# Ryan-Yanlong/DREAM-GNN

Measured on AMD Instinct MI355X. Metric: GCMC+FGCN SpMM edges/sec and achieved HBM GB/s at 1/2/4/8 MI355X, higher is better.
Workload: dtype f32

## Files before the change

dream_gnn_amd/csrc/dgmi_owned.hip:

```cpp
#include <hip/hip_runtime.h>
#include <stdint.h>

#include <map>
#include <mutex>
#include <utility>

#include "dgmi_owned_common.h"
#include "dgmi_sliced_common.h"

namespace dgmi {
namespace {

constexpr int kOwnedTouchChunk = 4;
constexpr int kOwnedTouchLead = 8;
constexpr int64_t kOwnedSpinTicks = 3000;
constexpr int64_t kOwnedMinRows = 32768;
constexpr int kOwnedLag = -1;

struct OwnedWork {
  int phase, task, slice, col_round;
  int64_t row0;
  int lds_row, rows;
};

__device__ __forceinline__ OwnedWork owned_decode(const OwnedPlan& pl, int64_t wg, int T, int k, int grp) {
  OwnedWork w;
  w.phase = k / T;
  w.task = k - w.phase * T;
  const OwnedPhase ph = owned_phase(pl, w.phase);
  w.slice = ph.slice;
  w.col_round = ph.col_round;
  const OwnedTask t = owned_task(pl, wg, ph.row_round, w.task, grp);
  w.row0 = t.row0;
  w.lds_row = t.lds_row;
  w.rows = t.rows;
  return w;
}

template <int LPR, int VALS, bool OFF32, int WAVES>
__global__ __launch_bounds__(kWave* WAVES, WAVES == kOwnedWaves ? 4 : 6) void spmm_owned_kernel(
    const int32_t* __restrict__ segptr, const int32_t* __restrict__ indices, const float* __restrict__ X, int64_t ldx,
    const float* __restrict__ dst_scale, float* __restrict__ Y, int64_t ldy, int64_t n_dst, int F, OwnedPlan pl,
    unsigned* __restrict__ arrive, int lag, int64_t spin_ticks, Epilogue ep) {
  constexpr bool MULT = VALS == 2;
  constexpr int kIdMask = MULT ? (int)kMultIdMask : 0x7fffffff;
  extern __shared__ float4 lds_rows[];
  const int lane = threadIdx.x & (kWave - 1);
  const int wave = threadIdx.x >> 6;
  const int grp = lane / LPR, glane = lane % LPR, gbase = grp * LPR;
  const int64_t wg = blockIdx.x;
  const int T = owned_wg_tasks(pl, wg);
  if (T == 0) return;
  int* done = reinterpret_cast<int*>(lds_rows + (size_t)pl.round_rows * LPR);
  int* phase_cnt = done + pl.tasks;
  int* counter = phase_cnt + pl.phases;
  int* open = counter + 1;
  for (int i = threadIdx.x; i < pl.tasks + pl.phases + 2; i += blockDim.x) done[i] = 0;
  __syncthreads();
  const int total = pl.phases * T;
  const int label = (int)(blockIdx.x & 7u);

  if (wave == WAVES - 1) {
    const unsigned n_label = (unsigned)((pl.active - label + 7) >> 3);
    const unsigned* my_arrive = arrive + (size_t)label * pl.phases;
    const int chunks_per_phase = (T + kOwnedTouchChunk - 1) / kOwnedTouchChunk, chunks = pl.phases * chunks_per_phase;
    const int last_gate = lag >= 0 ? pl.phases - 1 : 0;
    int keepalive = 0, touched = 0, opened = 0;
    bool waiting = false;
    uint64_t wait_start = 0;
    while (touched < chunks || opened < last_gate) {
      bool idle = true;
      const int next = __hip_atomic_load(counter, __ATOMIC_RELAXED, __HIP_MEMORY_SCOPE_WORKGROUP);
      if (touched < chunks) {
        const int P = touched / chunks_per_phase, t0 = (touched - P * chunks_per_phase) * kOwnedTouchChunk;
        if (P * T + t0 <= next + kOwnedTouchLead) {
          ++touched;
          idle = false;
          const OwnedPhase ph = owned_phase(pl, P);
          const int64_t in_round = owned_round_rows(pl, wg, ph.row_round);
          const int64_t lds_first = (int64_t)t0 * pl.G * pl.R;
          int64_t lds_last = lds_first + (int64_t)kOwnedTouchChunk * pl.G * pl.R;
          if (lds_last > in_round) lds_last = in_round;
          if (lds_first < lds_last) {
            const int32_t* sp_s = segptr + (int64_t)ph.slice * n_dst;
            const int64_t r_first = owned_task(pl, wg, ph.row_round, t0, 0).row0, r_last = r_first + (lds_last - lds_first);
            const int64_t rp = lane == 0 ? r_first : (lane == 1 ? r_last : r_first + (int64_t)(lane - 1) * 32);
            int v = 0;
            if (rp <= r_last) v = sp_s[rp];
            keepalive ^= v;
            const int e0 = __builtin_amdgcn_readlane(v, 0), e1 = __builtin_amdgcn_readlane(v, 1);
            for (int64_t p = (int64_t)e0 + (int64_t)lane * 32; p < e1; p += (int64_t)kWave * 32) keepalive ^= indices[p];
            asm volatile("" ::"v"(keepalive));
          }
        }
      }
      if (opened < last_gate) {
        const int P = opened + 1, need = P - 1 - lag;
        bool ok = need < 0 || __hip_atomic_load(&my_arrive[need], __ATOMIC_RELAXED, __HIP_MEMORY_SCOPE_AGENT) >= n_label;
        if (!ok && next >= P * T) {
          const uint64_t now = __builtin_amdgcn_s_memrealtime();
          if (!waiting) {
            waiting = true;
            wait_start = now;
          } else if (now - wait_start >= (uint64_t)spin_ticks) {
            ok = true;
          }
        }
        if (ok) {
          opened = P;
          waiting = false;
          idle = false;
          __hip_atomic_store(open, P, __ATOMIC_RELAXED, __HIP_MEMORY_SCOPE_WORKGROUP);
        }
      }
      if (idle) __builtin_amdgcn_s_sleep(2);
    }
    return;
  }

  auto grab = [&]() {
    int k = 0;
    if (lane == 0) k = __hip_atomic_fetch_add(counter, 1, __ATOMIC_RELAXED, __HIP_MEMORY_SCOPE_WORKGROUP);
    return __builtin_amdgcn_readfirstlane(k);
  };
  auto boundaries = [&](int k) {
    if (k >= total) return 0;
    const OwnedWork w = owned_decode(pl, wg, T, k, grp);
    if (w.rows == 0) return 0;
    return segptr[(int64_t)w.slice * n_dst + w.row0 + (glane < w.rows ? glane : w.rows)];
  };
  auto first_ids = [&](int my_b, int rows) {
    const int e_begin = __shfl(my_b, gbase, kWave), e_end = __shfl(my_b, gbase + rows, kWave);
    if (rows == 0 || e_begin >= e_end) return 0;
    return indices[e_begin + glane < e_end ? e_begin + glane : e_begin];
  };

  const uint32_t row_bytes = (uint32_t)ldx * 4u;
  int k = grab();
  int my_b = boundaries(k);
  int nxt_idx = k < total ? first_ids(my_b, owned_decode(pl, wg, T, k, grp).rows) : 0;
  while (k < total) {
    const OwnedWork w = owned_decode(pl, wg, T, k, grp);
    const int k_next = grab();
    const int next_b = boundaries(k_next);
    if (lag >= 0)
      while (__hip_atomic_load(open, __ATOMIC_RELAXED, __HIP_MEMORY_SCOPE_WORKGROUP) < w.phase) __builtin_amdgcn_s_sleep(1);
    while (__hip_atomic_load(&done[w.task], __ATOMIC_ACQUIRE, __HIP_MEMORY_SCOPE_WORKGROUP) < w.phase) __builtin_amdgcn_s_sleep(1);

    const int nr = w.rows;
    int col = (w.col_round * LPR + glane) * 4;
    const bool col_ok = col < F;
    if (!col_ok) col = 0;
    const float* Xc = X + col;
    const uint32_t col_bytes = (uint32_t)col * 4u;
    float4* slot = lds_rows + (size_t)w.lds_row * LPR + glane;
    auto commit = [&](int r, const float4& acc) {
      if (w.slice == 0) {
        slot[r * LPR] = acc;
        return;
      }
      float4 t = slot[r * LPR];
      t.x += acc.x;
      t.y += acc.y;
      t.z += acc.z;
      t.w += acc.w;
      slot[r * LPR] = t;
    };
    auto write_rows = [&]() {
      if (w.slice != kOwnedSlices - 1 || !col_ok) return;
      for (int r = 0; r < nr; ++r) {
        float4 t = slot[r * LPR];
        const int64_t row = w.row0 + r;
        if (dst_scale != nullptr) {
          const float d = dst_scale[row];
          t.x *= d;
          t.y *= d;
          t.z *= d;
          t.w *= d;
        }
        *reinterpret_cast<float4*>(Y + row * ldy + col) = epilogue4(ep, t, row, col);
      }
    };

    if (nr > 0) {
      const int e_begin = __shfl(my_b, gbase, kWave);
      const int e_end = __shfl(my_b, gbase + nr, kWave);
      int r = 0;
      int row_end = __shfl(my_b, gbase + 1, kWave);
      float4 acc = make_float4(0.f, 0.f, 0.f, 0.f);
      for (int base = e_begin; base < e_end; base += LPR) {
        const int n = min(LPR, e_end - base);
        const int my_idx = nxt_idx;
        if (base + LPR < e_end) {
          const int nb = base + LPR;
          nxt_idx = indices[nb + glane < e_end ? nb + glane : nb];
        }
        for (int j = 0; j < n; j += kUnroll) {
          float4 v[kUnroll];
          static_assert(kUnroll == 8 && kMultShift == 28, "eight 4-bit fields, each shifted down from bit 28");
          uint32_t mults = 0;
          auto mult = [&](int u) { return (float)(((mults >> (4 * u)) & (uint32_t)kMultMax) + 1u); };
#pragma unroll
          for (int u = 0; u < kUnroll; ++u) {
            int idx = __shfl(my_idx, gbase + j + u, kWave);
            if (MULT) {
              mults = (mults >> 4) | ((uint32_t)idx & ((uint32_t)kMultMax << kMultShift));
              idx &= kIdMask;
            }
            v[u] = ld_row<OFF32>(X, Xc, idx, ldx, row_bytes, col_bytes);
          }
          if (MULT) asm volatile("" : "+v"(mults));
          if (base + j + kUnroll <= row_end) {
#pragma unroll
            for (int u = 0; u < kUnroll; ++u) {
              if (MULT) {
                const float m = mult(u);
                acc.x = fmaf(m, v[u].x, acc.x);
                acc.y = fmaf(m, v[u].y, acc.y);
                acc.z = fmaf(m, v[u].z, acc.z);
                acc.w = fmaf(m, v[u].w, acc.w);
              } else {
                acc.x += v[u].x;
                acc.y += v[u].y;
                acc.z += v[u].z;
                acc.w += v[u].w;
              }
            }
            continue;
          }
#pragma unroll
          for (int u = 0; u < kUnroll; ++u) {
            const int p = base + j + u;
            if (p < e_end) {
              while (p >= row_end) {
                commit(r, acc);
                acc = make_float4(0.f, 0.f, 0.f, 0.f);
                ++r;
                row_end = __shfl(my_b, gbase + r + 1, kWave);
              }
              if (MULT) {
                const float m = mult(u);
                acc.x = fmaf(m, v[u].x, acc.x);
                acc.y = fmaf(m, v[u].y, acc.y);
                acc.z = fmaf(m, v[u].z, acc.z);
                acc.w = fmaf(m, v[u].w, acc.w);
              } else {
                acc.x += v[u].x;
                acc.y += v[u].y;
                acc.z += v[u].z;
                acc.w += v[u].w;
              }
            }
          }
        }
      }
      for (; r < nr; ++r) {
        commit(r, acc);
        acc = make_float4(0.f, 0.f, 0.f, 0.f);
      }
      write_rows();
    }
    nxt_idx = k_next < total ? first_ids(next_b, owned_decode(pl, wg, T, k_next, grp).rows) : 0;
    __builtin_amdgcn_wave_barrier();
    if (lane == 0) {
      __hip_atomic_store(&done[w.task], w.phase + 1, __ATOMIC_RELEASE, __HIP_MEMORY_SCOPE_WORKGROUP);
      if (lag >= 0) {
        const int finished = __hip_atomic_fetch_add(&phase_cnt[w.phase], 1, __ATOMIC_RELAXED, __HIP_MEMORY_SCOPE_WORKGROUP);
        if (finished == T - 1)
          __hip_atomic_fetch_add(&arrive[(size_t)label * pl.phases + w.phase], 1u, __ATOMIC_RELAXED, __HIP_MEMORY_SCOPE_AGENT);
      }
    }
    k = k_next;
    my_b = next_b;
  }
}

int device_cus() {
  static const int cus = [] {
    int dev = 0, n = 0;
    if (hipGetDevice(&dev) != hipSuccess || hipDeviceGetAttribute(&n, hipDeviceAttributeMultiprocessorCount, dev) != hipSuccess)
      return 0;
    return n;
  }();
  return cus;
}

int owned_class_form(const OwnedPlan& pl, bool id_mult, int64_t table_bytes) {
  if (pl.col_rounds == 1 && pl.row_rounds == 2 && !id_mult && table_bytes >= ((int64_t)16 << 20) && table_bytes <= ((int64_t)32 << 20))
    return 1;
  return 0;
}

bool owned_coresident(const void* kern, int threads, size_t lds, int wgs) {
  static std::mutex mu;
  static std::map<std::pair<const void*, size_t>, int> known;
  std::lock_guard<std::mutex> lock(mu);
  auto it = known.find({kern, lds});
  if (it == known.end()) {
    int n = 0;
    if (hipOccupancyMaxActiveBlocksPerMultiprocessor(&n, kern, threads, lds) != hipSuccess) {
      (void)hipGetLastError();
      n = 0;
    }
    it = known.emplace(std::make_pair(kern, lds), n).first;
  }
  return it->second >= wgs;
}

template <int LPR, int WAVES>
hipError_t launch_owned(const SlicedArgs& a, const OwnedPlan& pl, int64_t grid, bool off32, int lag, int64_t spin_ticks,
                        hipStream_t s, bool* resident) {
  constexpr int kWgsPerCu = WAVES == kOwnedWaves ? 1 : 2;
  unsigned* arrive = reinterpret_cast<unsigned*>(a.planes);
  *resident = true;
#define DGMI_OWNED(V, O)                                                                                                  \
  do {                                                                                                                    \
    if constexpr (kWgsPerCu > 1 && LPR == 8 && V == 2) {                                                                  \
      *resident = false;                                                                                                  \
      return hipSuccess;                                                                                                  \
    } else {                                                                                                              \
    auto kern = spmm_owned_kernel<LPR, V, O, WAVES>;                                                                      \
    static const hipError_t attr = hipFuncSetAttribute(reinterpret_cast<const void*>(kern),                               \
                                                       hipFuncAttributeMaxDynamicSharedMemorySize, (160 << 10) / kWgsPerCu); \
    if (attr != hipSuccess) return attr;                                                                                  \
    if (kWgsPerCu > 1 && !owned_coresident(reinterpret_cast<const void*>(kern), kWave * WAVES, pl.lds_bytes, kWgsPerCu)) { \
      *resident = false;                                                                                                  \
      return hipSuccess;                                                                                                  \
    }                                                                                                                     \
    if (lag >= 0) {                                                            \
      const hipError_t err = hipMemsetAsync(arrive, 0, sizeof(unsigned) * 8 * (size_t)pl.phases, s);                      \
      if (err != hipSuccess) return err;                                                                                  \
    }                                                                                                                     \
    hipLaunchKernelGGL(kern, dim3((unsigned)grid), dim3(kWave* WAVES), pl.lds_bytes, s, a.segptr, a.indices,              \
                       static_cast<const float*>(a.X), a.ldx, a.dst_scale, a.Y, a.ldy, a.n_dst, (int)a.F, pl, arrive, lag, \
                       spin_ticks, a.ep);                                                                                 \
    }                                                                                                                     \
  } while (0)
  if (a.id_mult) {
    if (off32) DGMI_OWNED(2, true); else DGMI_OWNED(2, false);
  } else {
    if (off32) DGMI_OWNED(0, true); else DGMI_OWNED(0, false);
  }
#undef DGMI_OWNED
  return hipGetLastError();
}

}

hipError_t spmm_owned_try(const SlicedArgs& a, hipStream_t s, bool* taken) {
  *taken = false;
  const Tuning& tune = tuning();
  if (tune.sliced_owned == 0) return hipSuccess;
  if (a.x_bytes != 4 || a.vals != nullptr || a.src_scale != nullptr || a.n_keep != 0 || a.n_slices != kOwnedSlices ||
      tune.sliced_chunk_rows > 0 || a.chunk_rows < a.n_dst || a.n_dst == 0 || a.F == 0)
    return hipSuccess;
  const int64_t grid = tune.sliced_owned_grid > 0 ? tune.sliced_owned_grid : device_cus();
  if (grid < 1) return hipSuccess;
  const int lpr = sliced_lpr(a.F, a.n_src, a.n_slices, a.n_dst, a.full_width, a.n_keep, a.x_bytes, tune.sliced_lpr);
  const OwnedPlan pl = owned_plan(a.n_dst, a.F, lpr, grid, tune.sliced_owned_rows, tune.sliced_owned_lds_rows);
  if (!pl.ok || pl.lds_bytes > (size_t)(160 << 10)) return hipSuccess;
  const auto arrive_fits = [&](const OwnedPlan& p) {
    return sizeof(unsigned) * 8 * (size_t)p.phases <= sizeof(float) * (size_t)a.n_slices * (size_t)a.n_dst * (size_t)a.ldp;
  };
  if (!arrive_fits(pl)) return hipSuccess;
  const int rule = a.n_dst < kOwnedMinRows ? 0 : owned_class_form(pl, a.id_mult, a.n_src * a.ldx * (int64_t)sizeof(float));
  if (tune.sliced_owned != 1 && rule == 0) return hipSuccess;
  const int form = tune.sliced_owned_wgs == 1 || tune.sliced_owned_wgs == 2 ? tune.sliced_owned_wgs : (rule == 2 ? 2 : 1);
  const bool off32 = !tune.sliced_no_off32 && (a.n_src * a.ldx + a.F) * 4 < ((int64_t)1 << 32);
  const int64_t spin = tune.sliced_owned_spin_ticks > 0 ? tune.sliced_owned_spin_ticks : kOwnedSpinTicks;
  const int lag = tune.sliced_owned_lag >= -1 ? tune.sliced_owned_lag : kOwnedLag;
  *taken = true;
  bool resident = true;
  if (form == 2) {
    const int64_t grid2 = tune.sliced_owned_grid > 0 ? grid : 2 * grid;
    const OwnedPlan pl2 = owned_plan(a.n_dst, a.F, lpr, grid2, tune.sliced_owned_rows, tune.sliced_owned_lds_rows, 2);
    if (pl2.ok && pl2.lds_bytes <= (size_t)(80 << 10) && arrive_fits(pl2)) {
      hipError_t err;
      switch (lpr) {
        case 8: err = launch_owned<8, kOwnedPairWaves>(a, pl2, grid2, off32, lag, spin, s, &resident); break;
        case 16: err = launch_owned<16, kOwnedPairWaves>(a, pl2, grid2, off32, lag, spin, s, &resident); break;
        case 32: err = launch_owned<32, kOwnedPairWaves>(a, pl2, grid2, off32, lag, spin, s, &resident); break;
        default: err = launch_owned<64, kOwnedPairWaves>(a, pl2, grid2, off32, lag, spin, s, &resident); break;
      }
      if (err != hipSuccess || resident) return err;
    }
  }
  switch (lpr) {
    case 8: return launch_owned<8, kOwnedWaves>(a, pl, grid, off32, lag, spin, s, &resident);
    case 16: return launch_owned<16, kOwnedWaves>(a, pl, grid, off32, lag, spin, s, &resident);
    case 32: return launch_owned<32, kOwnedWaves>(a, pl, grid, off32, lag, spin, s, &resident);
    default: return launch_owned<64, kOwnedWaves>(a, pl, grid, off32, lag, spin, s, &resident);
  }
}

}
```

dream_gnn_amd/csrc/dgmi_owned_common.h:

```cpp
#pragma once
#include <hip/hip_runtime.h>
#include <stddef.h>
#include <stdint.h>

namespace dgmi {

constexpr int kOwnedSlices = 8;
constexpr int kOwnedWaves = 16;
constexpr int kOwnedWorkers = kOwnedWaves - 1;
constexpr int kOwnedPairWaves = 12;
constexpr int64_t kOwnedLdsRowBytes = 144 << 10;
constexpr int kOwnedMaxPhases = 128;
constexpr int kOwnedPhaseTasks = 24;
constexpr int kOwnedMaxRows = 8;

struct OwnedPlan {
  bool ok;
  int lpr, G, R;
  int col_rounds, row_rounds, phases;
  int64_t wg_rows;
  int64_t active;
  int round_rows;
  int tasks;
  int64_t n_dst;
  size_t lds_bytes;
};

struct OwnedPhase {
  int col_round, row_round, slice;
};

struct OwnedTask {
  int64_t row0;
  int lds_row;
  int rows;
};

__host__ __device__ constexpr int owned_form_waves(int wgs_per_cu) { return wgs_per_cu == 2 ? kOwnedPairWaves : kOwnedWaves; }

__host__ __device__ inline OwnedPlan owned_plan(int64_t n_dst, int64_t F, int lpr, int64_t grid, int R_req, int64_t lds_rows_cap,
                                                int wgs_per_cu = 1) {
  OwnedPlan p{};
  p.ok = false;
  p.n_dst = n_dst;
  if (n_dst < 1 || F < 1 || grid < 1 || (wgs_per_cu != 1 && wgs_per_cu != 2) || (lpr != 8 && lpr != 16 && lpr != 32 && lpr != 64)) return p;
  p.lpr = lpr;
  p.G = 64 / lpr;
  p.col_rounds = (int)((F + 4 * lpr - 1) / (4 * lpr));
  p.wg_rows = (n_dst + grid - 1) / grid;
  p.active = (n_dst + p.wg_rows - 1) / p.wg_rows;
  int64_t fit = kOwnedLdsRowBytes / wgs_per_cu / (16 * lpr);
  if (lds_rows_cap > 0 && lds_rows_cap < fit) fit = lds_rows_cap;
  const int64_t rounds = (p.wg_rows + fit - 1) / fit;
  if (rounds * p.col_rounds * kOwnedSlices > kOwnedMaxPhases) return p;
  p.row_rounds = (int)rounds;
  p.round_rows = (int)((p.wg_rows + rounds - 1) / rounds);
  p.phases = p.col_rounds * p.row_rounds * kOwnedSlices;
  int R = R_req;
  if (R <= 0) {
    const int phase_tasks = (kOwnedPhaseTasks * (owned_form_waves(wgs_per_cu) - 1) + kOwnedWorkers / 2) / kOwnedWorkers;
    R = (p.round_rows + phase_tasks * p.G / 2) / (phase_tasks * p.G);
    if (R > kOwnedMaxRows) R = kOwnedMaxRows;
  }
  if (R > lpr - 1) R = lpr - 1;
  if (R < 1) R = 1;
  p.R = R;
  p.tasks = (p.round_rows + p.G * R - 1) / (p.G * R);
  p.lds_bytes = (size_t)p.round_rows * 16 * lpr + sizeof(int) * ((size_t)p.tasks + p.phases + 2);
  p.ok = true;
  return p;
}

__host__ __device__ inline int64_t owned_wg_rows(const OwnedPlan& p, int64_t wg) {
  const int64_t left = p.n_dst - wg * p.wg_rows;
  return left < 0 ? 0 : (left < p.wg_rows ? left : p.wg_rows);
}

__host__ __device__ inline int64_t owned_round_rows(const OwnedPlan& p, int64_t wg, int row_round) {
  const int64_t left = owned_wg_rows(p, wg) - (int64_t)row_round * p.round_rows;
  return left < 0 ? 0 : (left < p.round_rows ? left : p.round_rows);
}

__host__ __device__ inline int owned_wg_tasks(const OwnedPlan& p, int64_t wg) {
  int64_t rows = owned_wg_rows(p, wg);
  if (rows > p.round_rows) rows = p.round_rows;
  return (int)((rows + p.G * p.R - 1) / (p.G * p.R));
}

__host__ __device__ inline OwnedPhase owned_phase(const OwnedPlan& p, int phase) {
  const int cq = phase / kOwnedSlices;
  return OwnedPhase{cq / p.row_rounds, cq % p.row_rounds, phase % kOwnedSlices};
}

__host__ __device__ inline OwnedTask owned_task(const OwnedPlan& p, int64_t wg, int row_round, int task, int group) {
  const int64_t lds_row = ((int64_t)task * p.G + group) * p.R;
  int64_t rows = owned_round_rows(p, wg, row_round) - lds_row;
  rows = rows < 0 ? 0 : (rows < p.R ? rows : p.R);
  return OwnedTask{wg * p.wg_rows + (int64_t)row_round * p.round_rows + lds_row, (int)lds_row, (int)rows};
}

}
```

Measured before the change: 34.63 billion.

## Pipeline owned SpMM gathers with a sliding four-edge window and id prefetch

Replaces the per-LPR-chunk, eight-wide unrolled gather loop with a software-pipelined window of four row loads. Each slot is accumulated and then immediately reloaded, and the edge ids are prefetched two batches ahead. Scheduling barriers pin the order so memory requests stay in flight continuously, rather than being issued in bursts of eight and then drained. The id loads now fetch only W ids per batch, duplicated across lanes, which means more, smaller index loads. The change also routes two more id-multiplicity table-size classes to the alternate form.

New measurement: 36.37 billion (median of 6 runs). 5.0% higher.

```diff
diff --git a/dream_gnn_amd/csrc/dgmi_owned.hip b/dream_gnn_amd/csrc/dgmi_owned.hip
--- a/dream_gnn_amd/csrc/dgmi_owned.hip
+++ b/dream_gnn_amd/csrc/dgmi_owned.hip
@@ -129,16 +129,18 @@
     if (w.rows == 0) return 0;
     return segptr[(int64_t)w.slice * n_dst + w.row0 + (glane < w.rows ? glane : w.rows)];
   };
-  auto first_ids = [&](int my_b, int rows) {
+  auto first_ids = [&](int my_b, int rows, int batch) {
     const int e_begin = __shfl(my_b, gbase, kWave), e_end = __shfl(my_b, gbase + rows, kWave);
     if (rows == 0 || e_begin >= e_end) return 0;
-    return indices[e_begin + glane < e_end ? e_begin + glane : e_begin];
+    return indices[e_begin + owned_window_id_edge(batch, glane, e_end - e_begin)];
   };
+  static_assert(kOwnedWindowFirstBatches == 2, "nxt_idx and nxt_idx1");
 
   const uint32_t row_bytes = (uint32_t)ldx * 4u;
   int k = grab();
   int my_b = boundaries(k);
-  int nxt_idx = k < total ? first_ids(my_b, owned_decode(pl, wg, T, k, grp).rows) : 0;
+  int nxt_idx = k < total ? first_ids(my_b, owned_decode(pl, wg, T, k, grp).rows, 0) : 0;
+  int nxt_idx1 = k < total ? first_ids(my_b, owned_decode(pl, wg, T, k, grp).rows, 1) : 0;
   while (k < total) {
     const OwnedWork w = owned_decode(pl, wg, T, k, grp);
     const int k_next = grab();
@@ -188,69 +190,73 @@
       int r = 0;
       int row_end = __shfl(my_b, gbase + 1, kWave);
       float4 acc = make_float4(0.f, 0.f, 0.f, 0.f);
-      for (int base = e_begin; base < e_end; base += LPR) {
-        const int n = min(LPR, e_end - base);
-        const int my_idx = nxt_idx;
-        if (base + LPR < e_end) {
-          const int nb = base + LPR;
-          nxt_idx = indices[nb + glane < e_end ? nb + glane : nb];
-        }
-        for (int j = 0; j < n; j += kUnroll) {
-          float4 v[kUnroll];
-          static_assert(kUnroll == 8 && kMultShift == 28, "eight 4-bit fields, each shifted down from bit 28");
-          uint32_t mults = 0;
-          auto mult = [&](int u) { return (float)(((mults >> (4 * u)) & (uint32_t)kMultMax) + 1u); };
+      if (e_begin < e_end) {
+        constexpr int W = kOwnedWindow;
+        static_assert(W <= 8 && kMultShift == 28 && LPR % W == 0, "at most eight 4-bit multiplicity fields, shifted down from bit 28");
+        const int L = e_end - e_begin;
+        float4 v[W];
+        int idx[W];
+        uint32_t mults = 0, mults_in = 0;
+        auto read_ids = [&](int batch_idx) {
 #pragma unroll
-          for (int u = 0; u < kUnroll; ++u) {
-            int idx = __shfl(my_idx, gbase + j + u, kWave);
+          for (int u = 0; u < W; ++u) {
+            int id = __shfl(batch_idx, gbase + u, kWave);
             if (MULT) {
-              mults = (mults >> 4) | ((uint32_t)idx & ((uint32_t)kMultMax << kMultShift));
-              idx &= kIdMask;
+              mults_in = (mults_in >> 4) | ((uint32_t)id & ((uint32_t)kMultMax << kMultShift));
+              id &= kIdMask;
             }
-            v[u] = ld_row<OFF32>(X, Xc, idx, ldx, row_bytes, col_bytes);
-          }
-          if (MULT) asm volatile("" : "+v"(mults));
-          if (base + j + kUnroll <= row_end) {
+            idx[u] = id;
+          }
+          if (MULT) asm volatile("" : "+v"(mults_in));
+        };
+        auto add = [&](int u) {
+          if (MULT) {
+            const float m = (float)(((mults >> (32 - 4 * W)) & (uint32_t)kMultMax) + 1u);
+            mults >>= 4;
+            acc.x = fmaf(m, v[u].x, acc.x);
+            acc.y = fmaf(m, v[u].y, acc.y);
+            acc.z = fmaf(m, v[u].z, acc.z);
+            acc.w = fmaf(m, v[u].w, acc.w);
+          } else {
+            acc.x += v[u].x;
+            acc.y += v[u].y;
+            acc.z += v[u].z;
+            acc.w += v[u].w;
+          }
+        };
+        auto rows_before = [&](int p) {
+          while (p >= row_end) {
+            commit(r, acc);
+            acc = make_float4(0.f, 0.f, 0.f, 0.f);
+            ++r;
+            row_end = __shfl(my_b, gbase + r + 1, kWave);
+          }
+        };
+        read_ids(nxt_idx);
+        int ids = nxt_idx1;
 #pragma unroll
-            for (int u = 0; u < kUnroll; ++u) {
-              if (MULT) {
-                const float m = mult(u);
-                acc.x = fmaf(m, v[u].x, acc.x);
-                acc.y = fmaf(m, v[u].y, acc.y);
-                acc.z = fmaf(m, v[u].z, acc.z);
-                acc.w = fmaf(m, v[u].w, acc.w);
-              } else {
-                acc.x += v[u].x;
-                acc.y += v[u].y;
-                acc.z += v[u].z;
-                acc.w += v[u].w;
-              }
-            }
-            continue;
-          }
+        for (int u = 0; u < W; ++u) v[u] = ld_row<OFF32>(X, Xc, idx[u], ldx, row_bytes, col_bytes);
+        mults = mults_in;
+        __builtin_amdgcn_sched_barrier(0);
+        int p0 = e_begin;
+        for (int g = 0; p0 + W < e_end; ++g, p0 += W) {
+          read_ids(ids);
+          ids = indices[e_begin + owned_window_id_edge(owned_window_request_batch(g), glane, L)];
+          __builtin_amdgcn_sched_barrier(0);
 #pragma unroll
-          for (int u = 0; u < kUnroll; ++u) {
-            const int p = base + j + u;
-            if (p < e_end) {
-              while (p >= row_end) {
-                commit(r, acc);
-                acc = make_float4(0.f, 0.f, 0.f, 0.f);
-                ++r;
-                row_end = __shfl(my_b, gbase + r + 1, kWave);
-              }
-              if (MULT) {
-                const float m = mult(u);
-                acc.x = fmaf(m, v[u].x, acc.x);
-                acc.y = fmaf(m, v[u].y, acc.y);
-                acc.z = fmaf(m, v[u].z, acc.z);
-                acc.w = fmaf(m, v[u].w, acc.w);
-              } else {
-                acc.x += v[u].x;
-                acc.y += v[u].y;
-                acc.z += v[u].z;
-                acc.w += v[u].w;
-              }
-            }
+          for (int u = 0; u < W; ++u) {
+            rows_before(p0 + u);
+            add(u);
+            v[u] = ld_row<OFF32>(X, Xc, idx[u], ldx, row_bytes, col_bytes);
+            __builtin_amdgcn_sched_barrier(0);
+          }
+          mults = mults_in;
+        }
+#pragma unroll
+        for (int u = 0; u < W; ++u) {
+          if (p0 + u < e_end) {
+            rows_before(p0 + u);
+            add(u);
           }
         }
       }
@@ -260,7 +266,8 @@
       }
       write_rows();
     }
-    nxt_idx = k_next < total ? first_ids(next_b, owned_decode(pl, wg, T, k_next, grp).rows) : 0;
+    nxt_idx = k_next < total ? first_ids(next_b, owned_decode(pl, wg, T, k_next, grp).rows, 0) : 0;
+    nxt_idx1 = k_next < total ? first_ids(next_b, owned_decode(pl, wg, T, k_next, grp).rows, 1) : 0;
     __builtin_amdgcn_wave_barrier();
     if (lane == 0) {
       __hip_atomic_store(&done[w.task], w.phase + 1, __ATOMIC_RELEASE, __HIP_MEMORY_SCOPE_WORKGROUP);
@@ -286,8 +293,10 @@
 }
 
 int owned_class_form(const OwnedPlan& pl, bool id_mult, int64_t table_bytes) {
-  if (pl.col_rounds == 1 && pl.row_rounds == 2 && !id_mult && table_bytes >= ((int64_t)16 << 20) && table_bytes <= ((int64_t)32 << 20))
-    return 1;
+  const auto mib = [&](int64_t lo, int64_t hi) { return table_bytes >= (lo << 20) && table_bytes <= (hi << 20); };
+  if (pl.col_rounds == 1 && pl.row_rounds == 2 && !id_mult && mib(16, 32)) return 1;
+  if (pl.col_rounds == 2 && pl.row_rounds == 1 && id_mult && mib(48, 64)) return 1;
+  if (pl.col_rounds == 1 && pl.row_rounds == 1 && id_mult && mib(16, 32)) return 1;
   return 0;
 }
 
diff --git a/dream_gnn_amd/csrc/dgmi_owned_common.h b/dream_gnn_amd/csrc/dgmi_owned_common.h
--- a/dream_gnn_amd/csrc/dgmi_owned_common.h
+++ b/dream_gnn_amd/csrc/dgmi_owned_common.h
@@ -99,4 +99,16 @@
   return OwnedTask{wg * p.wg_rows + (int64_t)row_round * p.round_rows + lds_row, (int)lds_row, (int)rows};
 }
 
+constexpr int kOwnedWindow = 4;
+constexpr int kOwnedWindowFirstBatches = 2;
+
+__host__ __device__ constexpr int owned_window_groups(int L) { return (L + kOwnedWindow - 1) / kOwnedWindow; }
+
+__host__ __device__ constexpr int owned_window_issue_batch(int g) { return g + 1; }
+__host__ __device__ constexpr int owned_window_request_batch(int g) { return g + kOwnedWindowFirstBatches; }
+
+__host__ __device__ constexpr int owned_window_id_edge(int batch, int lane, int L) {
+  return batch * kOwnedWindow + lane % kOwnedWindow < L ? batch * kOwnedWindow + lane % kOwnedWindow : L - 1;
 }
+
+}
```
